# retrojetpacks/Gadget-Leicester

Hardware: AMD Instinct MI355X
Metric: particle-steps/sec (gravity+SPH) (higher is better)
Workload: dtype f64

## Files before the change

gadget-leicester_amd/csrc/ghip_gravity.hip:

```cpp
#include <cmath>

#include <hipcub/hipcub.hpp>

#include "ghip_walk.h"

__global__ void k_grav_finish(int nt, const int *__restrict__ tgt, const int *__restrict__ perm,
                              int n, double G, double comoving_fac, const double *__restrict__ pos,
                              const double *__restrict__ gravpm, double *__restrict__ oacc,
                              double *__restrict__ oldacc)
{
  int ti = blockIdx.x * blockDim.x + threadIdx.x;
  if(ti >= nt)
    return;
  int i = perm[tgt[ti]];
  double a0 = oacc[i], a1 = oacc[(size_t) n + i], a2 = oacc[2 * (size_t) n + i];
  if(comoving_fac != 0)
    {
      a0 += comoving_fac * pos[i];
      a1 += comoving_fac * pos[(size_t) n + i];
      a2 += comoving_fac * pos[2 * (size_t) n + i];
    }
  double b0 = a0, b1 = a1, b2 = a2;
  if(gravpm)
    {
// ... 146 lines not shown
extern "C" int ghip_ewald_init(ghip_ctx *ctx, double BoxSize)
{
  if(ctx)
    GHIP_JOIN(ctx);
  if(!ctx || !(BoxSize > 0))
    return ghip_fail(ctx, GHIP_EINVAL, "ghip_ewald_init: bad BoxSize");
  const int E1 = GHIP_EN + 1;
  const int nt = E1 * E1 * E1;
  GCHK(ghip_ensure(ctx, ctx->ewtab, (size_t) (nt + 2) * sizeof(double)));
  GCHK(ghip_ensure(ctx, ctx->ewbrick, (size_t) (GHIP_EW_DOUBLES + 2) * sizeof(double)));
  HIPCHK(hipMemsetAsync(ctx->ewbrick.p, 0, (size_t) (GHIP_EW_DOUBLES + 2) * sizeof(double), ctx->stream));
  k_ewald_table<<<cdiv(nt, 64), 64, 0, ctx->stream>>>(1.0 / (BoxSize * BoxSize),
                                                      P<double>(ctx->ewtab), P<double>(ctx->ewbrick));
  HIPCHK(hipGetLastError());
  ctx->ew_box = BoxSize;
  return GHIP_OK;
}

extern "C" int ghip_ewald_get_table(ghip_ctx *ctx, double *host)
{
  if(ctx)
    GHIP_JOIN(ctx);
  if(!ctx || !host || ctx->ew_box == 0)
    return ghip_fail(ctx, GHIP_EINVAL, "ghip_ewald_get_table: table not initialised");
  const int E1 = GHIP_EN + 1;
  const size_t nt = (size_t) E1 * E1 * E1;
  std::vector<double> tmp(nt);
  std::vector<double> brick((size_t) GHIP_EW_DOUBLES);
  HIPCHK(hipMemcpyAsync(tmp.data(), ctx->ewtab.p, nt * 8, hipMemcpyDeviceToHost, ctx->stream));
  HIPCHK(hipMemcpyAsync(brick.data(), ctx->ewbrick.p, brick.size() * 8, hipMemcpyDeviceToHost, ctx->stream));
  HIPCHK(ghip_stream_sync(ctx, ctx->stream));
  for(int i = 0; i < E1; i++)
    for(int j = 0; j < E1; j++)
      for(int k = 0; k < E1; k++)
        {
          const double v = tmp[((size_t) i * E1 + j) * E1 + k];
          if(brick[ghip_ew_offset(i, j, k / 3, k % 3)] != v ||
             (k % 3 == 0 && k > 0 && brick[ghip_ew_offset(i, j, k / 3 - 1, 3)] != v))
            return ghip_fail(ctx, GHIP_EDEVICE, "ewald table: the brick-tiled copy differs at (%d,%d,%d)",
                             i, j, k);
        }
  for(int i = 0; i < E1; i++)
    for(int j = 0; j < E1; j++)
      for(int k = 0; k < E1; k++)
        {
          size_t q = ((size_t) i * E1 + j) * E1 + k;
          host[q] = tmp[q];
          host[nt + q] = tmp[((size_t) j * E1 + i) * E1 + k];
          host[2 * nt + q] = tmp[((size_t) k * E1 + j) * E1 + i];
        }
  return GHIP_OK;
}

static int prepare_tables(ghip_ctx *ctx, const ghip_grav_params *p, int walk, GravK &k)
{
  k.theta = p->ErrTolTheta;
  k.errtol = p->ErrTolForceAcc;
  k.boxsize = p->BoxSize;
  k.boxhalf = 0.5 * p->BoxSize;
  k.periodic = p->periodic;
  k.unequal = p->unequal_softenings || ctx->adaptive_gravsoft;
  k.rcut = p->Rcut;
  k.rcut2 = p->Rcut * p->Rcut;
  k.asmthfac = (p->Asmth > 0) ? 0.5 / p->Asmth * (GHIP_NTAB / 3.0) : 0;
  k.fac_intp = (p->BoxSize > 0) ? 2 * GHIP_EN / p->BoxSize : 0;
  k.debug_steps = getenv("GHIP_DEBUG_STEPS") ? 1 : 0;
  k.k1875 = 1.875;
  if(ctx->dd.on)
    {
      int *w = ghip_errword(ctx, GHIP_ERRW_LET);
      HIPCHK(hipMemcpyToSymbolAsync(HIP_SYMBOL(d_walk_errw), &w, sizeof(w), 0, hipMemcpyHostToDevice,
                                    ctx->stream));
    }
  k.xcd_remap = getenv("GHIP_WALK_XCD") ? atoi(getenv("GHIP_WALK_XCD")) : 0;
  if(k.xcd_remap < 0)
    k.xcd_remap = 0;
  if(walk == GHIP_WALK_SHORTRANGE)
    {
      if(!(p->Asmth > 0) || !(p->Rcut > 0))
        return ghip_fail(ctx, GHIP_EINVAL, "shortrange walk needs Rcut, Asmth > 0");
      if(!ctx->srtab_ready)
        {
          float tab[GHIP_NTAB];
          for(int i = 0; i < GHIP_NTAB; i++)
            {
              double u = 3.0 / GHIP_NTAB * (i + 0.5);
              tab[i] = (float) (erfc(u) + 2.0 * u / sqrt(M_PI) * exp(-u * u));
            }
          GCHK(ghip_ensure(ctx, ctx->srtab, sizeof(tab)));
          HIPCHK(hipMemcpyAsync(ctx->srtab.p, tab, sizeof(tab), hipMemcpyHostToDevice,
                                ctx->stream));
          HIPCHK(ghip_stream_sync(ctx, ctx->stream));
          ctx->srtab_ready = true;
        }
    }
  if(walk == GHIP_WALK_EWALD)
    {
      if(!(p->BoxSize > 0))
        return ghip_fail(ctx, GHIP_EINVAL, "ewald walk needs BoxSize > 0");
      if(ctx->ew_box != p->BoxSize)
        GCHK(ghip_ewald_init(ctx, p->BoxSize));
    }
  return GHIP_OK;
}

int ghip_build_segments(ghip_ctx *ctx, TreeDev &t, bool walk_records)
{
  t.ns = 1;
  if(t.n == 0)
    return GHIP_OK;
  int ns = t.nelem / 2048;
  if(ns < 1)
    ns = 1;
  if(ns > 256)
    ns = 256;
  if(getenv("GHIP_WALK_SEGMENTS"))
    {
      int v = atoi(getenv("GHIP_WALK_SEGMENTS"));
      if(v >= 1 && v <= 4096)
        ns = v;
// ... 174 lines not shown
      ctx->plan_nb[kind] = nb;
      ctx->plan_ns[kind] = ns;
      ctx->plan_cur[kind] = cur ^ 1;
    }
  plan.nwaves = maxwaves;
  plan.wave_bucket = P<int>(b_wave);
  plan.woff = P<int>(b_woff);
  plan.nsub = P<int>(b_nsub);
  plan.steps_out = out;
  plan.started = nullptr;
  plan.started_at = 0;
  return GHIP_OK;
}

template <int MODE>
static void launch_walk(ghip_ctx *ctx, const TreeDev &t, const WalkSeg &sg, int nbuckets, int nt,
                        const int *tgt, const double *tx, const double *ty, const double *tz,
                        const double *tsoft, const double *toldacc, const GravK &k,
                        unsigned long long *counter, const WalkPlan &plan, const PartialBufs &pb,
                        hipStream_t stream)
{
  long long nthreads = (long long) plan.nwaves * 64;
  int bsize = 64;
  if(getenv("GHIP_WALK_BLOCK"))
    {
      int v = atoi(getenv("GHIP_WALK_BLOCK"));
      if(v == 64 || v == 128 || v == 256)
        bsize = v;
    }
  int blocks = cdiv(nthreads, bsize);
  blocks = (blocks + 7) & ~7;
  if(k.xcd_remap > 1)
    blocks = ((blocks + 8 * k.xcd_remap - 1) / (8 * k.xcd_remap)) * (8 * k.xcd_remap);
  WalkPlan pl = plan;
  if(pl.started)
    {
      static double frac = -1;
      if(frac < 0)
        frac = getenv("GHIP_HYDRO_TRIGGER_AT") ? atof(getenv("GHIP_HYDRO_TRIGGER_AT")) : 1.0;
      pl.started_at = (int) (frac * (blocks - 1));
      if(pl.started_at > blocks - 1 || pl.started_at < 0)
        pl.started_at = blocks - 1;
    }
  static int lds_env = -1;
  if(lds_env < 0)
    lds_env = getenv("GHIP_PAIR_NEWTON_LDS") ? atoi(getenv("GHIP_PAIR_NEWTON_LDS")) : 0;
  const int lds_n = lds_env > 0 ? lds_env : ctx->pair_lds;
  static int cap_min = -1;
  if(cap_min < 0)
    cap_min = getenv("GHIP_PAIR_CAP_MIN") ? atoi(getenv("GHIP_PAIR_CAP_MIN")) : 1536;
  static int lds_e = -1;
  if(lds_e < 0)
    lds_e = getenv("GHIP_PAIR_EWALD_LDS") ? atoi(getenv("GHIP_PAIR_EWALD_LDS")) : 0;
  const size_t dyn_lds =
    (MODE == GHIP_WALK_NEWTON && stream != ctx->stream && nbuckets >= cap_min)
      ? (size_t) lds_n
      : ((MODE == GHIP_WALK_EWALD && stream != ctx->stream && nbuckets >= cap_min) ? (size_t) lds_e : 0);
#define GHIP_LAUNCH_WALK(PER, UNEQ)                                                              \
  k_grav_walk<MODE, PER, UNEQ><<<blocks, bsize, dyn_lds, stream>>>(                                \
    t.nelem, P<WalkHot>(t.mq), P<WalkCold>(t.mq2), sg, nt, tgt, tx, ty, tz, tsoft, toldacc, k,     \
    P<float>(ctx->srtab), P<double>((UNEQ) && MODE == GHIP_WALK_EWALD ? ctx->ewbrick : ctx->ewtab),  \
    pb.ax, pb.ay, pb.az, pb.cost, getenv("GHIP_WALK_NOCOUNT") ? nullptr : counter,                  \
    P<unsigned long long>(ctx->rslots) + (counter - P<unsigned long long>(ctx->cslots)), pl)
  static int brick_env = -2;
  if(brick_env == -2)
    brick_env = getenv("GHIP_EW_BRICK") ? atoi(getenv("GHIP_EW_BRICK")) : -1;
  const bool brick = brick_env >= 0 ? brick_env != 0 : true;
  const bool uneq = (MODE == GHIP_WALK_EWALD) ? brick : (bool) k.unequal;
  if(k.periodic && uneq)
    GHIP_LAUNCH_WALK(true, true);
  else if(k.periodic)
    GHIP_LAUNCH_WALK(true, false);
  else if(uneq)
    GHIP_LAUNCH_WALK(false, true);
  else
    GHIP_LAUNCH_WALK(false, false);
#undef GHIP_LAUNCH_WALK
}

static void launch_walk_any(ghip_ctx *ctx, int walk, const TreeDev &t, const WalkSeg &sg,
                            int nbuckets, int nt, const int *tgt, const double *tx,
                            const double *ty, const double *tz, const double *tsoft,
                            const double *toldacc, const GravK &k, unsigned long long *counter,
                            const WalkPlan &plan, const PartialBufs &pb, hipStream_t stream)
{
  if(walk == GHIP_WALK_NEWTON)
    launch_walk<GHIP_WALK_NEWTON>(ctx, t, sg, nbuckets, nt, tgt, tx, ty, tz, tsoft, toldacc, k,
                                  counter, plan, pb, stream);
  else if(walk == GHIP_WALK_SHORTRANGE)
    launch_walk<GHIP_WALK_SHORTRANGE>(ctx, t, sg, nbuckets, nt, tgt, tx, ty, tz, tsoft, toldacc, k,
                                      counter, plan, pb, stream);
  else
    launch_walk<GHIP_WALK_EWALD>(ctx, t, sg, nbuckets, nt, tgt, tx, ty, tz, tsoft, toldacc, k,
                                 counter, plan, pb, stream);
}

static void shard_slice(const ghip_ctx *ctx, int nt, int *lo, int *cnt)
{
  int per;
  ghip_shard_range(nt, ctx->shard_n, ctx->shard_rank, lo, cnt, &per);
}

struct WalkJob
{
  int walk;
  GravK k;
  WalkSeg sg;
  WalkPlan plan;
  PartialBufs pb;
  int nbuckets;
  unsigned long long *counter;
};

static int prepare_job(ghip_ctx *ctx, const ghip_grav_params *p, int walk, int nt, int slot,
                       WalkJob &J, hipStream_t plan_on = nullptr)
{
  hipStream_t ps = plan_on ? plan_on : ctx->stream;
  J.walk = walk;
  GCHK(prepare_tables(ctx, p, walk, J.k));
  walk_layout(ctx->dyn_use ? ctx->dyn.tree : ctx->gt, nt, J.sg, &J.nbuckets, walk == GHIP_WALK_EWALD);
  GCHK(build_plan(ctx, walk == GHIP_WALK_EWALD ? 1 : 0, J.nbuckets, J.sg.ns, J.plan, slot, ps));
  GCHK(ensure_partials(ctx, J.plan.nwaves, slot, J.pb));
  J.counter = ghip_cslot(ctx, walk == GHIP_WALK_EWALD ? GHIP_CK_EWALD : GHIP_CK_NEWTON);
  HIPCHK(hipMemsetAsync(J.counter, 0, GHIP_CKIND_U64 * 8, ps));
  return GHIP_OK;
}

static int run_walk(ghip_ctx *ctx, const WalkJob &J, int nt, const int *tgt, hipStream_t st)
{
  int evi = (J.walk == GHIP_WALK_EWALD) ? 4 : 2;
  ctx->plan_writer[J.walk == GHIP_WALK_EWALD ? 1 : 0] = st;
  HIPCHK(hipEventRecord(ctx->evp[evi], st));
  launch_walk_any(ctx, J.walk, ctx->dyn_use ? ctx->dyn.tree : ctx->gt, J.sg, J.nbuckets, nt, tgt, P<double>(ctx->sx),
                  P<double>(ctx->sy), P<double>(ctx->sz), P<double>(ctx->ssoft),
                  P<double>(ctx->soldacc), J.k, J.counter, J.plan, J.pb, st);
  HIPCHK(hipGetLastError());
  HIPCHK(hipEventRecord(ctx->evp[evi + 1], st));
  return GHIP_OK;
}

static int combine_walk(ghip_ctx *ctx, const WalkJob &J, int nt, const int *tgt, hipStream_t st)
{
  k_combine_grav<<<cdiv(nt, 256), 256, 0, st>>>(
    nt, J.plan, tgt, P<int>(ctx->gt.perm), J.pb.ax, J.pb.ay, J.pb.az, J.pb.cost, ctx->n,
    P<double>(ctx->f[GHIP_F_GRAVACCEL]), P<int>(ctx->f[GHIP_F_GRAVCOST]),
    J.walk == GHIP_WALK_EWALD ? 1 : 0, J.k.debug_steps);
  HIPCHK(hipGetLastError());
  return GHIP_OK;
}

static int pair_balance(ghip_ctx *ctx)
{
  if(!ctx->pc_ev[3][3])
    {
      for(int i = 0; i < 4; i++)
        for(int j = 0; j < 4; j++)
          if(!ctx->pc_ev[i][j])
            HIPCHK(hipEventCreate(&ctx->pc_ev[i][j]));
      return GHIP_OK;
    }
  for(int i = 0; i < 4; i++)
    {
      if(ctx->pc_cap[i] == 0)
        continue;
      hipEvent_t *e = ctx->pc_ev[i];
      if(hipEventQuery(e[1]) != hipSuccess || hipEventQuery(e[3]) != hipSuccess)
        {
          (void) hipGetLastError();
          continue;
        }
      float tn = 0, te = 0;
      if(hipEventElapsedTime(&tn, e[0], e[1]) == hipSuccess && hipEventElapsedTime(&te, e[2], e[3]) == hipSuccess)
        {
          const int k = ctx->pc_cap[i] > 8192 ? 1 : 0;
          const float fe = ctx->pc_hyd[i] ? 1.1f : 1.0f;
          const float c = tn > fe * te ? tn : fe * te;
          ctx->pc_cost[k] = c;
          ctx->pc_age[k] = 0;
        }
      else
        (void) hipGetLastError();
      ctx->pc_cap[i] = 0;
    }
  ctx->pc_age[0]++;
  ctx->pc_age[1]++;
  const int cur = ctx->pair_lds > 8192 ? 1 : 0, oth = cur ^ 1;
  if(ctx->pc_cost[cur] < 0)
    return GHIP_OK;
  int want = cur;
  const bool close = ctx->pc_cost[oth] > 0 && ctx->pc_cost[oth] < 1.1f * ctx->pc_cost[cur] &&
                     ctx->pc_cost[cur] < 1.1f * ctx->pc_cost[oth];
  if(ctx->pc_cost[oth] < 0 || ctx->pc_age[oth] > (close ? 16 : 64))
    want = oth;
  else if(ctx->pc_cost[oth] < ctx->pc_cost[cur])
    want = oth;
  ctx->pair_lds = want ? 10240 : 8192;
  static int dbg = -1;
  if(dbg < 0)
    dbg = getenv("GHIP_PAIR_DEBUG") ? 1 : 0;
  if(dbg)
    fprintf(stderr, "[pair_balance] cost 8K %.3f (age %d)  10K %.3f (age %d)  -> %d\n", ctx->pc_cost[0],
            ctx->pc_age[0], ctx->pc_cost[1], ctx->pc_age[1], ctx->pair_lds);
  return GHIP_OK;
}

int ghip_gravity_impl(ghip_ctx *ctx, const ghip_grav_params *p, int walk)
{
  if(!ctx->gt.built)
    return ghip_fail(ctx, GHIP_EINVAL, "ghip_gravity: call ghip_tree_build first");
  if(walk < 0 || walk > GHIP_WALK_NEWTON_EWALD)
    return ghip_fail(ctx, GHIP_EINVAL, "ghip_gravity: unknown walk %d", walk);
  const bool pair = (walk == GHIP_WALK_NEWTON_EWALD);
  if(pair && !p->periodic)
    return ghip_fail(ctx, GHIP_EINVAL, "ghip_gravity: the Newton+Ewald pair needs periodic = 1");
  if(ctx->tree_unverified)
    {
      ghip_ctx::GravCall c;
      c.p = *p;
      c.walk = walk;
      ctx->grav_log.push_back(c);
    }
  GCHK(ghip_build_target_lists(ctx));
  hipStream_t st = ctx->stream;
  int n = ctx->n;
  int lo, nt;
  shard_slice(ctx, ctx->nt_grav, &lo, &nt);
  ghip_stats &S = ctx->stats;
  if(walk == GHIP_WALK_EWALD || pair)
    S.ewald_interactions = 0;
  if(walk != GHIP_WALK_EWALD)
    {
      S.grav_interactions = 0;
      S.grav_targets = nt;
    }
  if(nt == 0 || n == 0)
    return GHIP_OK;
  const int *tgt = P<int>(ctx->tg_grav) + lo;
  WalkJob A, E;
  hipStream_t pn = (pair && ctx->plan_writer[0] == ctx->stream3) ? ctx->stream3 : nullptr;
  hipStream_t pe = (pair && ctx->plan_writer[1] == ctx->stream2) ? ctx->stream2 : nullptr;
  if(getenv("GHIP_PLAN_ON_MAIN"))
    pn = nullptr;
  GCHK(prepare_job(ctx, p, pair ? GHIP_WALK_NEWTON : walk, nt, 0, A, pn));
  if(pair)
    GCHK(prepare_job(ctx, p, GHIP_WALK_EWALD, nt, 1, E, pe));

  GCHK(ghip_gather_f64_lim(ctx, ctx->gt.n, P<int>(ctx->gt.perm), P<double>(ctx->f[GHIP_F_OLDACC]),
                           n, P<double>(ctx->soldacc)));
  if(!pair)
    {
      GCHK(run_walk(ctx, A, nt, tgt, st));
      return combine_walk(ctx, A, nt, tgt, st);
    }
  hipStream_t sN = ctx->stream3, sE = ctx->stream2;
  HIPCHK(hipEventRecord(ctx->evx[0], st));
  HIPCHK(hipStreamWaitEvent(sN, ctx->evx[0], 0));
  HIPCHK(hipStreamWaitEvent(sE, ctx->evx[0], 0));
  GCHK(pair_balance(ctx));
  hipEvent_t *pc = ctx->pc_ev[ctx->pc_head];
  ctx->pc_cap[ctx->pc_head] = ctx->pair_lds;
  ctx->pc_hyd[ctx->pc_head] = 0;
  ctx->pc_head = (ctx->pc_head + 1) & 3;
  HIPCHK(hipEventRecord(pc[0], sN));
  GCHK(run_walk(ctx, A, nt, tgt, sN));
  HIPCHK(hipEventRecord(pc[1], sN));
  unsigned int *started = &ghip_words(ctx)->pair_started;
  HIPCHK(hipMemsetAsync(started, 0, 4, sE));
  E.plan.started = started;
  HIPCHK(hipEventRecord(pc[2], sE));
  GCHK(run_walk(ctx, E, nt, tgt, sE));
  HIPCHK(hipEventRecord(pc[3], sE));
  HIPCHK(hipEventRecord(ctx->evx[3], sE));
  if(A.k.debug_steps || E.k.debug_steps || getenv("GHIP_PAIR_TWO_COMBINES"))
    {
      GCHK(combine_walk(ctx, A, nt, tgt, sN));
// ... 200 lines not shown
```

gadget-leicester_amd/csrc/ghip_walk.h:

```cpp
#pragma once
#include "ghip_internal.h"
#include "ghip_count.h"

#ifndef GHIP_WALK_WAVES
#define GHIP_WALK_WAVES 8
#endif
#ifndef GHIP_WALK_OPT
#define GHIP_WALK_OPT 15
#endif


struct GravK
{
  double theta;
  double errtol;
  double boxsize, boxhalf;
  int periodic, unequal;
  int debug_steps;
  int xcd_remap;
  double rcut, rcut2, asmthfac;
  double fac_intp;
  double k1875;
};

__device__ int *d_walk_errw = nullptr;

#include "ghip_walkrec.h"

typedef double v16i __attribute__((ext_vector_type(8)));

struct __attribute__((aligned(8))) EwPair
{
  double lo, hi;
};
__device__ __forceinline__ EwPair d_ldpair(const double *p)
{
  return *reinterpret_cast<const EwPair *>(p);
}

__device__ __forceinline__ double d_f64(const v16i &v, int i)
{
  return v[i];
}
__device__ __forceinline__ int d_lo32(const v16i &v, int i)
{
  return __double2loint(v[i]);
}
__device__ __forceinline__ int d_hi32(const v16i &v, int i)
{
  return __double2hiint(v[i]);
}

__device__ __forceinline__ unsigned int d_rec_off(int e)
{
  return (unsigned int) __builtin_amdgcn_readfirstlane(e) << 6;
}
template <class T>
__device__ __forceinline__ void d_load1(const T *__restrict__ base, int e, v16i &R)
{
  const unsigned int off = d_rec_off(e);
  asm volatile("s_load_dwordx16 %0, %1, %2\n\ts_waitcnt lgkmcnt(0)" : "=s"(R) : "s"(base), "s"(off) : "memory");
}
template <class T>
__device__ __forceinline__ void d_load2(const T *__restrict__ base, int ea, v16i &A, int eb, v16i &B)
{
  const unsigned int oa = d_rec_off(ea), ob = d_rec_off(eb);
  asm volatile("s_load_dwordx16 %0, %2, %3\n\ts_load_dwordx16 %1, %2, %4\n\ts_waitcnt lgkmcnt(0)"
               : "=&s"(A), "=&s"(B)
               : "s"(base), "s"(oa), "s"(ob)
               : "memory");
}
template <class T>
__device__ __forceinline__ void d_touch_next(const T *__restrict__ base, unsigned int off, int &scratch)
{
  asm volatile("s_load_dword %0, %1, %2 offset:0x40" : "=s"(scratch) : "s"(base), "s"(off) : "memory");
// ... 115 lines not shown
      const unsigned int ck = ((((unsigned int) k * 43u) >> 7) * 13u + (unsigned int) k) * 8u;
      const unsigned int ci = ((((unsigned int) i * 43u) >> 7) * 13u + (unsigned int) i) * 8u;
      const char *tb = reinterpret_cast<const char *>(tab);
#define EW_LD(off) d_ldpair(reinterpret_cast<const double *>(tb + (off)))
      x00 = EW_LD(ai + bj + ck), x01 = EW_LD(ai + bj1 + ck), x10 = EW_LD(ai1 + bj + ck),
      x11 = EW_LD(ai1 + bj1 + ck);
      y00 = EW_LD(aj + bi + ck), y01 = EW_LD(aj + bi1 + ck), y10 = EW_LD(aj1 + bi + ck),
      y11 = EW_LD(aj1 + bi1 + ck);
      z00 = EW_LD(ak + bj + ci), z01 = EW_LD(ak + bj1 + ci), z10 = EW_LD(ak1 + bj + ci),
      z11 = EW_LD(ak1 + bj1 + ci);
#undef EW_LD
    }
  fx = sx * (x00.lo * f1 + x00.hi * f2 + x01.lo * f3 + x01.hi * f4 + x10.lo * f5 + x10.hi * f6 +
             x11.lo * f7 + x11.hi * f8);
  fy = sy * (y00.lo * f1 + y00.hi * f2 + y10.lo * f3 + y10.hi * f4 + y01.lo * f5 + y01.hi * f6 +
             y11.lo * f7 + y11.hi * f8);
  fz = sz * (z00.lo * f1 + z10.lo * f2 + z01.lo * f3 + z11.lo * f4 + z00.hi * f5 + z10.hi * f6 +
             z01.hi * f7 + z11.hi * f8);
}

struct WalkLane
{
  double pos_x, pos_y, pos_z, h_i, aold;
  double h2;
  double k15;
  double acc_x, acc_y, acc_z;
  int nint;
};

__device__ __forceinline__ double d_nearest1(double x, double boxsize, double boxhalf)
{
  return (fabs(x) > boxhalf) ? x - copysign(boxsize, x) : x;
}

__device__ __forceinline__ double d_nearest1_masked(double x, double boxsize, double boxhalf)
{
  if(fabs(x) > boxhalf)
    {
      x -= copysign(boxsize, x);
      asm volatile("" : "+v"(x));
    }
  return x;
}

typedef unsigned long long lmask;
#define D_BAL(cond) __builtin_amdgcn_ballot_w64(cond)
#define D_LANE(mask) __builtin_amdgcn_inverse_ballot_w64(mask)

__device__ __forceinline__ void d_skip_to(int &my_skip, int skip)
{
  asm volatile("v_max_i32 %0, %1, %0" : "+v"(my_skip) : "s"(skip));
}

template <int MODE, bool PERIODIC, bool UNEQUAL, bool OWNED, bool REL>
__device__ __forceinline__ int d_walk_element(int e, const v16i &H,
                                              const WalkCold *__restrict__ cold, const GravK &p,
                                              const float *__restrict__ srtab,
                                              const double *__restrict__ ewtab, WalkLane &W,
                                              int &my_skip)
{
  const double ex = d_f64(H, 0), ey = d_f64(H, 1), ez = d_f64(H, 2), mass = d_f64(H, 3);
  const double mlen2 = d_f64(H, 4), len2 = d_f64(H, 5);
  const int skip = d_lo32(H, 6), pidx = d_hi32(H, 6);
  const double aux = d_f64(H, 7);
  const lmask act = D_BAL(e >= my_skip);
  int next;

  double dx = ex - W.pos_x, dy = ey - W.pos_y, dz = ez - W.pos_z;
  double r2;
  if((GHIP_WALK_OPT & 1) && (MODE == GHIP_WALK_EWALD || PERIODIC))
    {
      r2 = dx * dx + dy * dy + dz * dz;
      if(D_BAL(r2 >= p.boxhalf * p.boxhalf) != 0)
        {
          if(D_LANE(D_BAL(fabs(dx) > p.boxhalf)))
            {
              dx -= copysign(p.boxsize, dx);
              asm volatile("" : "+v"(dx));
            }
          if(D_LANE(D_BAL(fabs(dy) > p.boxhalf)))
            {
              dy -= copysign(p.boxsize, dy);
              asm volatile("" : "+v"(dy));
            }
          if(D_LANE(D_BAL(fabs(dz) > p.boxhalf)))
            {
              dz -= copysign(p.boxsize, dz);
              asm volatile("" : "+v"(dz));
            }
          r2 = dx * dx + dy * dy + dz * dz;
        }
    }
  else if(MODE == GHIP_WALK_EWALD || PERIODIC)
    {
      const lmask wx = D_BAL(fabs(dx) > p.boxhalf), wy = D_BAL(fabs(dy) > p.boxhalf),
                  wz = D_BAL(fabs(dz) > p.boxhalf);
      if((wx | wy | wz) != 0)
        {
          if(D_LANE(wx))
            {
              dx -= copysign(p.boxsize, dx);
              asm volatile("" : "+v"(dx));
            }
          if(D_LANE(wy))
            {
              dy -= copysign(p.boxsize, dy);
              asm volatile("" : "+v"(dy));
            }
          if(D_LANE(wz))
            {
              dz -= copysign(p.boxsize, dz);
              asm volatile("" : "+v"(dz));
// ... 87 lines not shown
        }
      if(MODE != GHIP_WALK_EWALD && UNEQUAL)
        {
          const double ms = fabs(aux);
          const lmask up = act & ~drop & ~open & D_BAL(h < ms);
          if(up != 0)
            {
              if(D_LANE(up))
                {
                  h = ms;
                  h2 = ms * ms;
                }
              if(aux < 0)
                open |= up & D_BAL(r2 < ms * ms);
            }
        }
      interact = act & ~drop & ~open;
      if(!((GHIP_WALK_OPT & 4) && OWNED && MODE == GHIP_WALK_NEWTON) || (interact & D_BAL(r2 < h2)) != 0)
        if(D_LANE(interact | drop))
          d_skip_to(my_skip, skip);
      next = skip;
      if(open != 0)
        {
          next = e + 1;
          if(skip == next)
            {
              int *w = *(int *volatile *) &d_walk_errw;
              if(w)
                *(volatile int *) w = 1;
            }
        }
    }

  if(OWNED && MODE == GHIP_WALK_NEWTON && (interact & D_BAL(r2 < h2)) == 0)
    {
      const int counted = pidx & 1;
      const int sk = skip;
      if(D_LANE(interact))
        {
          const double fac = (GHIP_WALK_OPT & 8) ? d_mass_over_r3(mass, r2, W.k15, p.k1875)
                                                 : d_mass_over_r3(mass, r2);
          W.acc_x += dx * fac;
          W.acc_y += dy * fac;
          W.acc_z += dz * fac;
          if(GHIP_WALK_OPT & 2)
            W.nint += counted;
          else
            W.nint += (mass > 0) ? 1 : 0;
          if(GHIP_WALK_OPT & 4)
            d_skip_to(my_skip, sk);
        }
      return next;
    }
  if(OWNED && D_LANE(interact))
    {
      if(MODE == GHIP_WALK_EWALD)
        {
          double fx, fy, fz;
          d_ewald_interp<UNEQUAL>(ewtab, p.fac_intp, dx, dy, dz, fx, fy, fz);
          W.acc_x += mass * fx;
          W.acc_y += mass * fy;
          W.acc_z += mass * fz;
          W.nint++;
        }
      else
        {
          double r;
          double fac = d_grav_fac(mass, r2, h, h2, r);
          if(MODE == GHIP_WALK_SHORTRANGE)
            {
              int tabindex = (int) (p.asmthfac * r);
              if(tabindex < GHIP_NTAB)
                {
                  fac *= srtab[tabindex];
                  W.acc_x += dx * fac;
                  W.acc_y += dy * fac;
                  W.acc_z += dz * fac;
                  W.nint++;
                }
            }
          else
            {
              W.acc_x += dx * fac;
              W.acc_y += dy * fac;
              W.acc_z += dz * fac;
              if(mass > 0)
                W.nint++;
            }
        }
    }
  return next;
}

struct WalkPlan
{
  int nwaves;
  const int *__restrict__ wave_bucket;
  const int *__restrict__ woff;
  const int *__restrict__ nsub;
  unsigned int *__restrict__ steps_out;
  unsigned int *started;
  int started_at;
};

struct SegCursor
{
  int kseg;
  int e, s1;
};

template <int MODE, bool PERIODIC, bool UNEQUAL, bool REL>
__device__ __forceinline__ bool d_enter_segment(SegCursor &c, int stride, const WalkSeg &sg,
                                                const WalkHot *__restrict__ hot,
                                                const WalkCold *__restrict__ cold, const GravK &p,
                                                const float *__restrict__ srtab,
                                                const double *__restrict__ ewtab, bool valid,
                                                WalkLane &W, int &my_skip, unsigned int &steps)
{
  while(c.kseg < sg.ns)
    {
      const int s0 = __builtin_amdgcn_readfirstlane(sg.start[c.kseg]);
      c.s1 = __builtin_amdgcn_readfirstlane(sg.start[c.kseg + 1]);
      my_skip = valid ? 0 : 0x7fffffff;
      const int na = __builtin_amdgcn_readfirstlane(sg.nanc[c.kseg]);
      for(int a = 0; a < na; a++)
        {
          int ea = __builtin_amdgcn_readfirstlane(sg.anc[c.kseg * GHIP_MAXANC + a]);
          v16i H;
          d_load1(hot, ea, H);
          d_walk_element<MODE, PERIODIC, UNEQUAL, false, REL>(ea, H, cold, p, srtab, ewtab, W, my_skip);
          steps++;
        }
      int first = d_wave_min_i32(my_skip);
      c.e = __builtin_amdgcn_readfirstlane(first > s0 ? first : s0);
      if(c.e < c.s1)
        return true;
      c.kseg += stride;
    }
  return false;
}

template <int MODE, bool PERIODIC, bool UNEQUAL, bool REL>
__device__ __forceinline__ void d_walk_run(const WalkSeg &sg, int sub, const WalkHot *__restrict__ hot,
                                           const WalkCold *__restrict__ cold, const GravK &p,
                                           const float *__restrict__ srtab,
                                           const double *__restrict__ ewtab, bool valid, WalkLane &W,
                                           unsigned int &steps)
{
  if(MODE != GHIP_WALK_EWALD)
    {
      SegCursor A;
      int skipA = 0;
      A.kseg = sub;
      const int stride = sg.nsub;
      bool liveA = d_enter_segment<MODE, PERIODIC, UNEQUAL, REL>(A, stride, sg, hot, cold, p, srtab,
                                                            ewtab, valid, W, skipA, steps);
      int t1 = 0, t2 = 0;
      while(liveA)
        {
          v16i HA;
          const unsigned int offA = d_rec_off(A.e);
          d_load1_touch(hot, offA, HA, t1, t2);
          d_touch_next(hot, offA, t1);
          d_touch(hot, d_lo32(HA, 6), t2);
          steps++;
          A.e = __builtin_amdgcn_readfirstlane(
            d_walk_element<MODE, PERIODIC, UNEQUAL, true, REL>(A.e, HA, cold, p, srtab, ewtab, W, skipA));
          if(A.e >= A.s1)
            {
              d_drain_touch(t1, t2);
              A.kseg += stride;
              liveA = d_enter_segment<MODE, PERIODIC, UNEQUAL, REL>(A, stride, sg, hot, cold, p, srtab,
                                                               ewtab, valid, W, skipA, steps);
            }
        }
      d_drain_touch(t1, t2);
    }
  else
    {
      SegCursor A, B;
      int skipA = 0, skipB = 0;
      A.kseg = sub;
      B.kseg = sub + sg.nsub;
      const int stride = 2 * sg.nsub;
      bool liveA = d_enter_segment<MODE, PERIODIC, UNEQUAL, REL>(A, stride, sg, hot, cold, p, srtab, ewtab, valid,
                                                   W, skipA, steps);
      bool liveB = d_enter_segment<MODE, PERIODIC, UNEQUAL, REL>(B, stride, sg, hot, cold, p, srtab, ewtab, valid,
                                                   W, skipB, steps);
      while(liveA && liveB)
        {
          v16i HA, HB;
          d_load2(hot, A.e, HA, B.e, HB);
          steps += 2;
          A.e = __builtin_amdgcn_readfirstlane(
            d_walk_element<MODE, PERIODIC, UNEQUAL, true, REL>(A.e, HA, cold, p, srtab, ewtab, W, skipA));
          B.e = __builtin_amdgcn_readfirstlane(
            d_walk_element<MODE, PERIODIC, UNEQUAL, true, REL>(B.e, HB, cold, p, srtab, ewtab, W, skipB));
          if(A.e >= A.s1)
            {
              A.kseg += stride;
              liveA = d_enter_segment<MODE, PERIODIC, UNEQUAL, REL>(A, stride, sg, hot, cold, p, srtab, ewtab,
                                                      valid, W, skipA, steps);
            }
          if(B.e >= B.s1)
            {
              B.kseg += stride;
              liveB = d_enter_segment<MODE, PERIODIC, UNEQUAL, REL>(B, stride, sg, hot, cold, p, srtab, ewtab,
                                                      valid, W, skipB, steps);
            }
        }
      if(liveB)
        {
          A = B;
          skipA = skipB;
          liveA = true;
        }
      while(liveA)
        {
          v16i HA;
          d_load1(hot, A.e, HA);
          steps++;
          A.e = __builtin_amdgcn_readfirstlane(
            d_walk_element<MODE, PERIODIC, UNEQUAL, true, REL>(A.e, HA, cold, p, srtab, ewtab, W, skipA));
          if(A.e >= A.s1)
            {
              A.kseg += stride;
              liveA = d_enter_segment<MODE, PERIODIC, UNEQUAL, REL>(A, stride, sg, hot, cold, p, srtab, ewtab,
                                                      valid, W, skipA, steps);
            }
        }
    }

}

template <int MODE, bool PERIODIC, bool UNEQUAL>
__global__ void __launch_bounds__(GHIP_BLOCK) __attribute__((amdgpu_waves_per_eu(MODE == GHIP_WALK_EWALD ? 4 : GHIP_WALK_WAVES, 8)))
k_grav_walk(int nelem, const WalkHot *__restrict__ hot, const WalkCold *__restrict__ cold,
            WalkSeg sg, int nt, const int *__restrict__ tgt, const double *__restrict__ tx,
            const double *__restrict__ ty, const double *__restrict__ tz,
            const double *__restrict__ tsoft, const double *__restrict__ toldacc, GravK p,
            const float *__restrict__ srtab, const double *__restrict__ ewtab,
            double *__restrict__ pax, double *__restrict__ pay, double *__restrict__ paz,
            int *__restrict__ pcost, unsigned long long *__restrict__ counter,
            unsigned long long *__restrict__ acc, WalkPlan plan)
{
  const int lane = threadIdx.x & 63;
  if(plan.started && blockIdx.x == plan.started_at && threadIdx.x == 0)
    __hip_atomic_store(plan.started, 1u, __ATOMIC_RELEASE, __HIP_MEMORY_SCOPE_SYSTEM);
  const int per_xcd = gridDim.x >> 3;
  int lblock = blockIdx.x;
  if(p.xcd_remap == 1)
    lblock = (blockIdx.x & 7) * per_xcd + (blockIdx.x >> 3);
  else if(p.xcd_remap > 1)
    {
      const int j = blockIdx.x >> 3, x = blockIdx.x & 7, G = p.xcd_remap;
      lblock = ((j / G) * 8 + x) * G + (j % G);
    }
  const int wave = __builtin_amdgcn_readfirstlane((lblock * (int) blockDim.x + threadIdx.x) >> 6);
  if(wave >= plan.nwaves)
    return;
  const int bucket = __builtin_amdgcn_readfirstlane(plan.wave_bucket[wave]);
  if(bucket < 0 || bucket * 64 >= nt)
    return;
  const int sub = wave - __builtin_amdgcn_readfirstlane(plan.woff[bucket]);
  sg.nsub = __builtin_amdgcn_readfirstlane(plan.nsub[bucket]);
  const int ti = bucket * 64 + lane;
  const bool valid = ti < nt;
  const int s = valid ? (tgt ? tgt[ti] : ti) : 0;

  WalkLane W;
  W.pos_x = W.pos_y = W.pos_z = 0;
  W.h_i = 1;
  W.aold = 0;
  W.h2 = 1;
  if(valid)
    {
      W.pos_x = tx[s];
      W.pos_y = ty[s];
      W.pos_z = tz[s];
      W.h_i = tsoft[s];
      W.aold = p.errtol * toldacc[s];
      W.h2 = W.h_i * W.h_i;
    }
  W.acc_x = W.acc_y = W.acc_z = 0;
  W.nint = 0;
  W.k15 = 1.5;
  asm volatile("" : "+v"(W.k15));
  unsigned int steps = 0;

  if(p.theta == 0)
    d_walk_run<MODE, PERIODIC, UNEQUAL, true>(sg, sub, hot, cold, p, srtab, ewtab, valid, W, steps);
  else
    d_walk_run<MODE, PERIODIC, UNEQUAL, false>(sg, sub, hot, cold, p, srtab, ewtab, valid, W, steps);

  if(valid)
    {
      const size_t o = (size_t) wave * 64 + lane;
      pax[o] = W.acc_x;
      pay[o] = W.acc_y;
      paz[o] = W.acc_z;
      pcost[o] = p.debug_steps ? (int) steps : W.nint;
    }
  unsigned long long tot = d_wave_sum_u64((unsigned long long) W.nint);
  if(lane == 0 && tot && counter)
    {
      d_count(counter, 0, tot);
      d_count(acc, 0, tot);
    }
  if(lane == 0)
    {
      if(counter)
        {
          d_count(counter, 1, (unsigned long long) steps);
          d_count(acc, 1, (unsigned long long) steps);
        }
      atomicAdd(plan.steps_out + bucket, steps);
    }
}

__global__ void k_plan_nsub(int nb, int ns, int sbase, const unsigned int *__restrict__ steps_prev,
                            int nprev, int *__restrict__ nsub)
{
  __shared__ unsigned long long part[4];
  unsigned long long tot = 0;
  if(nprev > 0)
    {
      for(int k = threadIdx.x; k < nprev; k += blockDim.x)
        tot += steps_prev[k];
      for(int o = 32; o > 0; o >>= 1)
        tot += __shfl_xor(tot, o);
      if((threadIdx.x & 63) == 0)
        part[threadIdx.x >> 6] = tot;
      __syncthreads();
      tot = part[0] + part[1] + part[2] + part[3];
    }
  int b = blockIdx.x * blockDim.x + threadIdx.x;
  if(b >= nb)
    return;
  int s = ns < sbase ? ns : sbase;
  if(b < nprev && tot > 0)
    {
      double mean = (double) tot / (double) nprev;
      s = (int) ((double) sbase * (double) steps_prev[b] / mean) + 1;
      s = s < 2 ? 2 : s;
      s = s > 64 ? 64 : s;
      if(s > ns)
        s = ns;
    }
  nsub[b] = s < 1 ? 1 : s;
}

__global__ void k_plan_fill(int nb, const int *__restrict__ nsub, const int *__restrict__ woff,
                            int maxwaves, int *__restrict__ wave_bucket,
                            unsigned int *__restrict__ steps_out, int *__restrict__ errword)
{
  int b = blockIdx.x * blockDim.x + threadIdx.x;
  if(b >= nb)
    return;
  int o = woff[b], s = nsub[b];
  if(o + s > maxwaves)
    *(volatile int *) errword = 1;
  for(int q = 0; q < s; q++)
    if(o + q < maxwaves)
      wave_bucket[o + q] = b;
  steps_out[b] = 0;
}

struct SegTables
{
  int ntab;
// ... 176 lines not shown
```

Baseline: 81.38 million.

## Batch sparse Ewald interactions into a per-wave LDS queue for dense evaluation

When fewer than a threshold number of lanes in a wave need an Ewald correction for a tree element, the per-lane interaction (dx,dy,dz,mass) is pushed into a per-wave LDS queue instead of running the costly Ewald table interpolation under a sparse mask. The queue is drained when near full, with all lanes interpolating queued entries, and each lane then accumulates its own results by following a linked list in LDS. This is meant to raise SIMD utilisation of the divergent Ewald correction. In exchange it adds LDS usage per wave, lowers the pair-kernel LDS caps, and adds wave barriers and queue bookkeeping to the walk loop. It also restructures the two-stream walk loop so the queue can be drained between steps.

```diff
diff --git a/gadget-leicester_amd/csrc/ghip_gravity.hip b/gadget-leicester_amd/csrc/ghip_gravity.hip
--- a/gadget-leicester_amd/csrc/ghip_gravity.hip
+++ b/gadget-leicester_amd/csrc/ghip_gravity.hip
@@ -222,6 +222,16 @@
   return GHIP_OK;
 }
 
+static int ew_sparse_t()
+{
+  const char *s = getenv("GHIP_EW_SPARSE");
+  if(s && atoi(s) == 0)
+    return 0;
+  const char *t = getenv("GHIP_EW_SPARSE_T");
+  const int v = t ? atoi(t) : 16;
+  return v < 1 ? 1 : (v > 65 ? 65 : v);
+}
+
 static int prepare_tables(ghip_ctx *ctx, const ghip_grav_params *p, int walk, GravK &k)
 {
   k.theta = p->ErrTolTheta;
@@ -236,6 +246,10 @@
   k.fac_intp = (p->BoxSize > 0) ? 2 * GHIP_EN / p->BoxSize : 0;
   k.debug_steps = getenv("GHIP_DEBUG_STEPS") ? 1 : 0;
   k.k1875 = 1.875;
+  k.ew_t = (walk == GHIP_WALK_EWALD) ? ew_sparse_t() : 0;
+  k.ew_lim = 64 - 2 * (k.ew_t - 1);
+  if(k.ew_lim < 0)
+    k.ew_lim = 0;
   if(ctx->dd.on)
     {
       int *w = ghip_errword(ctx, GHIP_ERRW_LET);
@@ -516,10 +530,12 @@
   static int lds_e = -1;
   if(lds_e < 0)
     lds_e = getenv("GHIP_PAIR_EWALD_LDS") ? atoi(getenv("GHIP_PAIR_EWALD_LDS")) : 0;
-  const size_t dyn_lds =
+  size_t dyn_lds =
     (MODE == GHIP_WALK_NEWTON && stream != ctx->stream && nbuckets >= cap_min)
       ? (size_t) lds_n
       : ((MODE == GHIP_WALK_EWALD && stream != ctx->stream && nbuckets >= cap_min) ? (size_t) lds_e : 0);
+  if(MODE == GHIP_WALK_EWALD && k.ew_t > 0 && dyn_lds < (size_t) (bsize / 64) * GHIP_EWQ_BYTES)
+    dyn_lds = (size_t) (bsize / 64) * GHIP_EWQ_BYTES;
 #define GHIP_LAUNCH_WALK(PER, UNEQ)                                                              \
   k_grav_walk<MODE, PER, UNEQ><<<blocks, bsize, dyn_lds, stream>>>(                                \
     t.nelem, P<WalkHot>(t.mq), P<WalkCold>(t.mq2), sg, nt, tgt, tx, ty, tz, tsoft, toldacc, k,     \
@@ -613,8 +629,19 @@
   return GHIP_OK;
 }
 
+static void pair_caps(int *lo, int *hi)
+{
+  const bool q = ew_sparse_t() > 0;
+  *lo = q ? 7680 : 8192;
+  *hi = q ? 7680 : 10240;
+}
+
 static int pair_balance(ghip_ctx *ctx)
 {
+  int cap_lo, cap_hi;
+  pair_caps(&cap_lo, &cap_hi);
+  if(ctx->pair_lds != cap_lo && ctx->pair_lds != cap_hi)
+    ctx->pair_lds = cap_hi;
   if(!ctx->pc_ev[3][3])
     {
       for(int i = 0; i < 4; i++)
@@ -636,7 +663,7 @@
       float tn = 0, te = 0;
       if(hipEventElapsedTime(&tn, e[0], e[1]) == hipSuccess && hipEventElapsedTime(&te, e[2], e[3]) == hipSuccess)
         {
-          const int k = ctx->pc_cap[i] > 8192 ? 1 : 0;
+          const int k = ctx->pc_cap[i] >= cap_hi ? 1 : 0;
           const float fe = ctx->pc_hyd[i] ? 1.1f : 1.0f;
           const float c = tn > fe * te ? tn : fe * te;
           ctx->pc_cost[k] = c;
@@ -648,7 +675,7 @@
     }
   ctx->pc_age[0]++;
   ctx->pc_age[1]++;
-  const int cur = ctx->pair_lds > 8192 ? 1 : 0, oth = cur ^ 1;
+  const int cur = ctx->pair_lds >= cap_hi ? 1 : 0, oth = cur ^ 1;
   if(ctx->pc_cost[cur] < 0)
     return GHIP_OK;
   int want = cur;
@@ -658,7 +685,7 @@
     want = oth;
   else if(ctx->pc_cost[oth] < ctx->pc_cost[cur])
     want = oth;
-  ctx->pair_lds = want ? 10240 : 8192;
+  ctx->pair_lds = want ? cap_hi : cap_lo;
   static int dbg = -1;
   if(dbg < 0)
     dbg = getenv("GHIP_PAIR_DEBUG") ? 1 : 0;
@@ -685,6 +712,19 @@
       ctx->grav_log.push_back(c);
     }
   GCHK(ghip_build_target_lists(ctx));
+#ifdef GHIP_EW_HIST
+  if(ctx->cslots.p)
+    {
+      unsigned long long h[GHIP_CKIND_U64], b[8] = {0, 0, 0, 0, 0, 0, 0, 0};
+      HIPCHK(hipDeviceSynchronize());
+      HIPCHK(hipMemcpy(h, ghip_cslot(ctx, GHIP_CK_EWALD), sizeof(h), hipMemcpyDeviceToHost));
+      for(int s = 0; s < GHIP_CSLOTS; s++)
+        for(int w = 0; w < 8; w++)
+          b[w] += h[s * GHIP_CSLOT_U64 + 2 + w];
+      fprintf(stderr, "[ew_hist] lanes 1-8 %llu 9-16 %llu 17-24 %llu 25-32 %llu 33-40 %llu 41-48 %llu 49-56 %llu 57-64 %llu\n",
+              b[0], b[1], b[2], b[3], b[4], b[5], b[6], b[7]);
+    }
+#endif
   hipStream_t st = ctx->stream;
   int n = ctx->n;
   int lo, nt;
diff --git a/gadget-leicester_amd/csrc/ghip_walk.h b/gadget-leicester_amd/csrc/ghip_walk.h
--- a/gadget-leicester_amd/csrc/ghip_walk.h
+++ b/gadget-leicester_amd/csrc/ghip_walk.h
@@ -21,6 +21,8 @@
   double rcut, rcut2, asmthfac;
   double fac_intp;
   double k1875;
+  int ew_t;
+  int ew_lim;
 };
 
 __device__ int *d_walk_errw = nullptr;
@@ -242,12 +244,77 @@
   asm volatile("v_max_i32 %0, %1, %0" : "+v"(my_skip) : "s"(skip));
 }
 
+#define GHIP_EWQ_DOUBLES 320
+#define GHIP_EWQ_BYTES (GHIP_EWQ_DOUBLES * 8)
+extern __shared__ double d_ewq[];
+
+struct EwQueue
+{
+  int n;
+  int base;
+  int tail;
+#ifdef GHIP_EW_HIST
+  unsigned int hist;
+#endif
+};
+
+__device__ __forceinline__ void d_ewq_fence()
+{
+  __builtin_amdgcn_fence(__ATOMIC_ACQ_REL, "wavefront");
+  __builtin_amdgcn_wave_barrier();
+}
+
+__device__ __forceinline__ void d_ewq_push(EwQueue &Q, lmask mask, double dx, double dy, double dz,
+                                           double mass)
+{
+  const int s = Q.n + (int) __builtin_amdgcn_mbcnt_hi((unsigned int) (mask >> 32),
+                                                      __builtin_amdgcn_mbcnt_lo((unsigned int) mask, 0u));
+  double *q = d_ewq + Q.base;
+  q[s] = dx;
+  q[s + 64] = dy;
+  q[s + 128] = dz;
+  q[s + 192] = mass;
+  reinterpret_cast<int *>(q + 256)[Q.tail] = s;
+  Q.tail = s;
+}
+
+template <bool BRICK>
+__device__ __forceinline__ void d_ewq_drain(EwQueue &Q, const double *__restrict__ ewtab, double fac_intp,
+                                            int lane, WalkLane &W)
+{
+  double *q = d_ewq + Q.base;
+  int *qw = reinterpret_cast<int *>(q + 256);
+  qw[Q.tail] = -1;
+  d_ewq_fence();
+  if(lane < Q.n)
+    {
+      const double dx = q[lane], dy = q[lane + 64], dz = q[lane + 128], mass = q[lane + 192];
+      double fx, fy, fz;
+      d_ewald_interp<BRICK>(ewtab, fac_intp, dx, dy, dz, fx, fy, fz);
+      q[lane] = mass * fx;
+      q[lane + 64] = mass * fy;
+      q[lane + 128] = mass * fz;
+    }
+  d_ewq_fence();
+  for(int s = qw[64 + lane]; s >= 0;)
+    {
+      W.acc_x += q[s];
+      W.acc_y += q[s + 64];
+      W.acc_z += q[s + 128];
+      const int nx = qw[s];
+      s = nx > s ? nx : -1;
+    }
+  d_ewq_fence();
+  Q.tail = 64 + lane;
+  Q.n = 0;
+}
+
 template <int MODE, bool PERIODIC, bool UNEQUAL, bool OWNED, bool REL>
 __device__ __forceinline__ int d_walk_element(int e, const v16i &H,
                                               const WalkCold *__restrict__ cold, const GravK &p,
                                               const float *__restrict__ srtab,
                                               const double *__restrict__ ewtab, WalkLane &W,
-                                              int &my_skip)
+                                              int &my_skip, EwQueue &Q)
 {
   const double ex = d_f64(H, 0), ey = d_f64(H, 1), ez = d_f64(H, 2), mass = d_f64(H, 3);
   const double mlen2 = d_f64(H, 4), len2 = d_f64(H, 5);
@@ -441,6 +508,27 @@
         }
       return next;
     }
+  if(OWNED && MODE == GHIP_WALK_EWALD)
+    {
+      const int cnt = __builtin_popcountll(interact);
+#ifdef GHIP_EW_HIST
+      if(cnt)
+        Q.hist += (((cnt - 1) >> 3) ==
+                   (int) __builtin_amdgcn_mbcnt_hi(~0u, __builtin_amdgcn_mbcnt_lo(~0u, 0u)))
+                    ? 1u
+                    : 0u;
+#endif
+      if(cnt < p.ew_t && Q.n + cnt <= 64)
+        {
+          if(D_LANE(interact))
+            {
+              d_ewq_push(Q, interact, dx, dy, dz, mass);
+              W.nint++;
+            }
+          Q.n += cnt;
+          return next;
+        }
+    }
   if(OWNED && D_LANE(interact))
     {
       if(MODE == GHIP_WALK_EWALD)
@@ -504,7 +592,8 @@
                                                 const WalkCold *__restrict__ cold, const GravK &p,
                                                 const float *__restrict__ srtab,
                                                 const double *__restrict__ ewtab, bool valid,
-                                                WalkLane &W, int &my_skip, unsigned int &steps)
+                                                WalkLane &W, int &my_skip, unsigned int &steps,
+                                                EwQueue &Q)
 {
   while(c.kseg < sg.ns)
     {
@@ -517,7 +606,7 @@
           int ea = __builtin_amdgcn_readfirstlane(sg.anc[c.kseg * GHIP_MAXANC + a]);
           v16i H;
           d_load1(hot, ea, H);
-          d_walk_element<MODE, PERIODIC, UNEQUAL, false, REL>(ea, H, cold, p, srtab, ewtab, W, my_skip);
+          d_walk_element<MODE, PERIODIC, UNEQUAL, false, REL>(ea, H, cold, p, srtab, ewtab, W, my_skip, Q);
           steps++;
         }
       int first = d_wave_min_i32(my_skip);
@@ -534,7 +623,7 @@
                                            const WalkCold *__restrict__ cold, const GravK &p,
                                            const float *__restrict__ srtab,
                                            const double *__restrict__ ewtab, bool valid, WalkLane &W,
-                                           unsigned int &steps)
+                                           unsigned int &steps, int lane, EwQueue &Q)
 {
   if(MODE != GHIP_WALK_EWALD)
     {
@@ -543,7 +632,7 @@
       A.kseg = sub;
       const int stride = sg.nsub;
       bool liveA = d_enter_segment<MODE, PERIODIC, UNEQUAL, REL>(A, stride, sg, hot, cold, p, srtab,
-                                                            ewtab, valid, W, skipA, steps);
+                                                            ewtab, valid, W, skipA, steps, Q);
       int t1 = 0, t2 = 0;
       while(liveA)
         {
@@ -554,13 +643,13 @@
           d_touch(hot, d_lo32(HA, 6), t2);
           steps++;
           A.e = __builtin_amdgcn_readfirstlane(
-            d_walk_element<MODE, PERIODIC, UNEQUAL, true, REL>(A.e, HA, cold, p, srtab, ewtab, W, skipA));
+            d_walk_element<MODE, PERIODIC, UNEQUAL, true, REL>(A.e, HA, cold, p, srtab, ewtab, W, skipA, Q));
           if(A.e >= A.s1)
             {
               d_drain_touch(t1, t2);
               A.kseg += stride;
               liveA = d_enter_segment<MODE, PERIODIC, UNEQUAL, REL>(A, stride, sg, hot, cold, p, srtab,
-                                                               ewtab, valid, W, skipA, steps);
+                                                               ewtab, valid, W, skipA, steps, Q);
             }
         }
       d_drain_touch(t1, t2);
@@ -573,49 +662,58 @@
       B.kseg = sub + sg.nsub;
       const int stride = 2 * sg.nsub;
       bool liveA = d_enter_segment<MODE, PERIODIC, UNEQUAL, REL>(A, stride, sg, hot, cold, p, srtab, ewtab, valid,
-                                                   W, skipA, steps);
+                                                   W, skipA, steps, Q);
       bool liveB = d_enter_segment<MODE, PERIODIC, UNEQUAL, REL>(B, stride, sg, hot, cold, p, srtab, ewtab, valid,
-                                                   W, skipB, steps);
-      while(liveA && liveB)
-        {
-          v16i HA, HB;
-          d_load2(hot, A.e, HA, B.e, HB);
-          steps += 2;
-          A.e = __builtin_amdgcn_readfirstlane(
-            d_walk_element<MODE, PERIODIC, UNEQUAL, true, REL>(A.e, HA, cold, p, srtab, ewtab, W, skipA));
-          B.e = __builtin_amdgcn_readfirstlane(
-            d_walk_element<MODE, PERIODIC, UNEQUAL, true, REL>(B.e, HB, cold, p, srtab, ewtab, W, skipB));
-          if(A.e >= A.s1)
-            {
-              A.kseg += stride;
-              liveA = d_enter_segment<MODE, PERIODIC, UNEQUAL, REL>(A, stride, sg, hot, cold, p, srtab, ewtab,
-                                                      valid, W, skipA, steps);
-            }
-          if(B.e >= B.s1)
-            {
-              B.kseg += stride;
-              liveB = d_enter_segment<MODE, PERIODIC, UNEQUAL, REL>(B, stride, sg, hot, cold, p, srtab, ewtab,
-                                                      valid, W, skipB, steps);
-            }
-        }
-      if(liveB)
-        {
-          A = B;
-          skipA = skipB;
-          liveA = true;
-        }
-      while(liveA)
-        {
-          v16i HA;
-          d_load1(hot, A.e, HA);
-          steps++;
-          A.e = __builtin_amdgcn_readfirstlane(
-            d_walk_element<MODE, PERIODIC, UNEQUAL, true, REL>(A.e, HA, cold, p, srtab, ewtab, W, skipA));
-          if(A.e >= A.s1)
-            {
-              A.kseg += stride;
-              liveA = d_enter_segment<MODE, PERIODIC, UNEQUAL, REL>(A, stride, sg, hot, cold, p, srtab, ewtab,
-                                                      valid, W, skipA, steps);
+                                                   W, skipB, steps, Q);
+      for(;;)
+        {
+          const bool two = liveA && liveB;
+          if(!two && liveB)
+            {
+              A = B;
+              skipA = skipB;
+              liveA = true;
+              liveB = false;
+            }
+          if(Q.n > (liveA ? p.ew_lim : 0))
+            d_ewq_drain<UNEQUAL>(Q, ewtab, p.fac_intp, lane, W);
+          if(!liveA)
+            break;
+          if(two)
+            {
+              v16i HA, HB;
+              d_load2(hot, A.e, HA, B.e, HB);
+              steps += 2;
+              A.e = __builtin_amdgcn_readfirstlane(
+                d_walk_element<MODE, PERIODIC, UNEQUAL, true, REL>(A.e, HA, cold, p, srtab, ewtab, W, skipA, Q));
+              B.e = __builtin_amdgcn_readfirstlane(
+                d_walk_element<MODE, PERIODIC, UNEQUAL, true, REL>(B.e, HB, cold, p, srtab, ewtab, W, skipB, Q));
+              if(A.e >= A.s1)
+                {
+                  A.kseg += stride;
+                  liveA = d_enter_segment<MODE, PERIODIC, UNEQUAL, REL>(A, stride, sg, hot, cold, p, srtab, ewtab,
+                                                                        valid, W, skipA, steps, Q);
+                }
+              if(B.e >= B.s1)
+                {
+                  B.kseg += stride;
+                  liveB = d_enter_segment<MODE, PERIODIC, UNEQUAL, REL>(B, stride, sg, hot, cold, p, srtab, ewtab,
+                                                                        valid, W, skipB, steps, Q);
+                }
+            }
+          else
+            {
+              v16i HA;
+              d_load1(hot, A.e, HA);
+              steps++;
+              A.e = __builtin_amdgcn_readfirstlane(
+                d_walk_element<MODE, PERIODIC, UNEQUAL, true, REL>(A.e, HA, cold, p, srtab, ewtab, W, skipA, Q));
+              if(A.e >= A.s1)
+                {
+                  A.kseg += stride;
+                  liveA = d_enter_segment<MODE, PERIODIC, UNEQUAL, REL>(A, stride, sg, hot, cold, p, srtab, ewtab,
+                                                                        valid, W, skipA, steps, Q);
+                }
             }
         }
     }
@@ -676,11 +774,18 @@
   W.k15 = 1.5;
   asm volatile("" : "+v"(W.k15));
   unsigned int steps = 0;
+  EwQueue Q;
+  Q.n = 0;
+  Q.base = __builtin_amdgcn_readfirstlane((int) (threadIdx.x >> 6) * GHIP_EWQ_DOUBLES);
+  Q.tail = 64 + lane;
+#ifdef GHIP_EW_HIST
+  Q.hist = 0;
+#endif
 
   if(p.theta == 0)
-    d_walk_run<MODE, PERIODIC, UNEQUAL, true>(sg, sub, hot, cold, p, srtab, ewtab, valid, W, steps);
+    d_walk_run<MODE, PERIODIC, UNEQUAL, true>(sg, sub, hot, cold, p, srtab, ewtab, valid, W, steps, lane, Q);
   else
-    d_walk_run<MODE, PERIODIC, UNEQUAL, false>(sg, sub, hot, cold, p, srtab, ewtab, valid, W, steps);
+    d_walk_run<MODE, PERIODIC, UNEQUAL, false>(sg, sub, hot, cold, p, srtab, ewtab, valid, W, steps, lane, Q);
 
   if(valid)
     {
@@ -705,6 +810,10 @@
         }
       atomicAdd(plan.steps_out + bucket, steps);
     }
+#ifdef GHIP_EW_HIST
+  if(MODE == GHIP_WALK_EWALD && lane < 8 && Q.hist && counter)
+    d_count(counter, 2 + lane, (unsigned long long) Q.hist);
+#endif
 }
 
 __global__ void k_plan_nsub(int nb, int ns, int sbase, const unsigned int *__restrict__ steps_prev,
```

New measurement: 81.87 million (median of 6 runs). No clear change (+0.6%).
